# luisdiaz1997/GPzoo

Hardware: AMD Instinct MI355X
Metric: ELBO evals/sec (L=32-latent evaluations, all GPUs) at M=2048 inducing, N=200000, L=32 latents/GPU x 1 GPU(s) (higher is better)
Workload: dtype f32; 1 GPU; BASELINE configs[2]: Slide-seq-shaped synthetic, N=200000 spots, M=2048, L=32 latents/GPU x 1 GPU(s), matern32, f32; latents_total=32, whitened=True, chunk=0, factor_dtype=f64

## Files before the change

gpzoo_amd/csrc/gemmw.hip:

```cpp
#include "gemmw.h"

#include "cov.h"


#include <cmath>
#include <mutex>
#include <type_traits>
#include <utility>

#ifndef GPZ_W_ABL
#define GPZ_W_ABL 0
#endif

namespace gpz {

typedef float f32x4 __attribute__((ext_vector_type(4)));

enum { WB_MEM = 0, WB_GEN = 1 };
enum { WA_DENSE = 0, WA_LOWER = 1, WA_UPPER = 2 };
enum { WE_STORE_STATS = 0,
       WE_STATS = 1,
       WE_STORE = 2,
       WE_STORE_COLSCALE = 3,
       WE_WBAR = 4,
       WE_KBAR = 5,
       WE_ADD_COLSCALE = 6 };

struct WParams {
  const float* A; int64_t lda, sA0;
  const float* B; int64_t ldb, sB0;
  const float* Z; int64_t MD;
  const float* X; int64_t nreal;
  const float* sigma; const float* ell;
  float* C; int64_t ldc, sC0;
  const float* mu; int64_t sMu;
  float* ps_sq; float* ps_mu; int64_t ncols;
  const float* colscale; const float* colvec; int64_t sCs;
  const float* rowvec; int64_t sRv;
  const float* aux;
  int64_t M;
  int L, nblk, mtw, nt, W, strips;
  int pair, colmajor;
  const int32_t* gate;
};

constexpr int W_BK = 16;

template <int TM, int TN, int BSRC, int D>
struct WLds {
  static constexpr int A_ELEMS = TM * W_BK;
  static constexpr int RPP = 256 / TN;
  static constexpr int PITCH = 256 + (RPP == 2 ? 8 : RPP == 1 ? 4 : 16);
  static constexpr int B_ELEMS = (W_BK / RPP) * PITCH;
  static constexpr int STAGE = A_ELEMS + B_ELEMS;
  static constexpr int ZB = 128 * D;
  static constexpr size_t bytes = sizeof(float) * (2 * STAGE + (BSRC == WB_GEN ? 2 * ZB : 0));
};

template <int TM, int TN, int BSRC, int ATRI, int EPI, int KIND, int D>
__global__ __launch_bounds__(64 * (TM / 128) * (TN / 32)) __attribute__((amdgpu_waves_per_eu(4, 4))) void gemmw_kernel(const WParams p) {
  constexpr int BK = W_BK;
  if (p.gate && *p.gate == 0) return;
  constexpr int WMW = TM / 128, WNW = TN / 32;
  constexpr int NW = WMW * WNW;
  static_assert(NW == 8 || NW == 16, "8 or 16 waves of 128 x 32");
  using G = WLds<TM, TN, BSRC, D>;
  constexpr int RPP = G::RPP, PITCH = G::PITCH;
  extern __shared__ __attribute__((aligned(1024))) char smem_raw[];
  float* const smem = reinterpret_cast<float*>(smem_raw);
  auto sA = [&](int buf) -> float* { return smem + buf * G::STAGE; };
  auto sB = [&](int buf) -> float* { return smem + buf * G::STAGE + G::A_ELEMS; };
  float* const sZ = smem + 2 * G::STAGE;
  auto addrB = [](int k, int n) { return (k / RPP) * PITCH + (k % RPP) * TN + n; };

  int tj, b0, leg_ti[2], nlegs = 1;
  {
    const int bid = blockIdx.x;
    const int x = bid & 7, s = bid >> 3;
    if (BSRC == WB_GEN) {
      const int ug = s / p.W, within = s - ug * p.W;
      const int u = ug * 8 + x;
      const int per_level = p.L * p.strips;
      if (u >= p.mtw * per_level) return;
      const int level = u / per_level, rem = u - level * per_level;
      leg_ti[0] = leg_ti[1] = (ATRI == WA_LOWER) ? p.mtw - 1 - level : level;
      b0 = rem / p.strips;
      tj = (rem - b0 * p.strips) * p.W + within;
    } else {
      const int per_unit = (p.pair ? (p.mtw + 1) >> 1 : p.mtw) * p.W;
      const int u = (s / per_unit) * 8 + x, within = s % per_unit;
      if (u >= p.L * p.strips) return;
      b0 = u / p.strips;
      const int nrow = p.pair ? (p.mtw + 1) >> 1 : p.mtw;
      const int pi = p.colmajor ? within % nrow : within / p.W, far = p.pair ? p.mtw - 1 - pi : pi;
      const int strip = u - b0 * p.strips, c0 = strip * p.nt / p.strips, c1 = (strip + 1) * p.nt / p.strips;
      tj = c0 + (p.colmajor ? within / nrow : within % p.W);
      if (tj >= c1) return;
      const bool long_first = ((s >> 5) & 1) == 0;
      leg_ti[0] = ((ATRI == WA_LOWER) == long_first) ? far : pi;
      leg_ti[1] = ((ATRI == WA_LOWER) == long_first) ? pi : far;
      nlegs = far == pi ? 1 : 2;
      if (!p.pair) leg_ti[0] = leg_ti[1] = (ATRI == WA_LOWER) ? p.mtw - 1 - pi : pi;
    }
    if (tj >= p.nt) return;
  }
  const int tid = threadIdx.x, lane = tid & 63;
  const int wave = __builtin_amdgcn_readfirstlane(tid >> 6);
  const int wn = wave % WNW;
  const int r = lane & 15, q = lane >> 4;
  const int Mp = p.nblk * 128;

  typedef __attribute__((address_space(3))) void lds_void;
  constexpr int NPA = TM / (16 * NW);
#if defined(__HIP_DEVICE_COMPILE__)
  const __amdgpu_buffer_rsrc_t a_rsrc = __builtin_amdgcn_make_buffer_rsrc(
      const_cast<float*>(p.A + b0 * p.sA0), 0, (int)(p.lda * Mp * sizeof(float)), 0x00020000);
  const __amdgpu_buffer_rsrc_t b_rsrc = __builtin_amdgcn_make_buffer_rsrc(
      const_cast<float*>(BSRC == WB_MEM ? p.B + b0 * p.sB0 : p.Z), 0,
      (int)((BSRC == WB_MEM ? p.ldb * Mp : p.MD) * sizeof(float)), 0x00020000);
#endif
  auto k_begin_of = [&](int ti) { return (ATRI == WA_UPPER) ? TM * ti : 0; };
  auto k_end_of = [&](int ti) { return (ATRI == WA_LOWER) ? min(TM * (ti + 1), Mp) : Mp; };
  int a_soff[NPA], b_soff = 0;
  auto gperm = [](int w) { const int t = (w >> 2) & 3; return (((t >> 1) ^ t) & 1) << 1 | (t >> 1); };
  const int a_voff = ((lane >> 2) * (int)p.lda + (((lane & 3) ^ gperm(lane >> 2)) * 4)) * (int)sizeof(float);
  const int b_voff = ((lane / (TN / 4)) * (int)p.ldb + (lane % (TN / 4)) * 4) * (int)sizeof(float);
  bool abl_first = true;
  auto stage_load = [&](int buf) __attribute__((always_inline)) {
    if ((GPZ_W_ABL & 2) && !abl_first) return;
    abl_first = false;
#if defined(__HIP_DEVICE_COMPILE__)
#pragma unroll
    for (int h = 0; h < NPA; ++h) {
      __builtin_amdgcn_raw_ptr_buffer_load_lds(a_rsrc, (lds_void*)(sA(buf) + (NPA * wave + h) * 256), 16, a_voff, a_soff[h], 0, 0);
      a_soff[h] += BK * (int)sizeof(float);
    }
    if constexpr (BSRC == WB_MEM) {
      constexpr int NPB = (W_BK / RPP) / NW;
      static_assert(BSRC != WB_MEM || (NPB * NW * RPP == W_BK && NPB >= 1), "whole B pieces per wave");
#pragma unroll
      for (int h = 0; h < NPB; ++h)
        __builtin_amdgcn_raw_ptr_buffer_load_lds(b_rsrc, (lds_void*)(sB(buf) + (wave + NW * h) * PITCH), 16, b_voff,
                                                 b_soff + h * NW * RPP * (int)p.ldb * (int)sizeof(float), 0, 0);
      b_soff += BK * (int)p.ldb * (int)sizeof(float);
    }
#endif
  };
  auto tile_begin = [&](int ti) __attribute__((always_inline)) {
    const int kb = k_begin_of(ti);
#pragma unroll
    for (int h = 0; h < NPA; ++h) {
      int row = ti * TM + (NPA * wave + h) * 16;
      while (row >= Mp) row -= 128;
      a_soff[h] = (row * (int)p.lda + kb) * (int)sizeof(float);
    }
    b_soff = ((kb + RPP * wave) * (int)p.ldb + tj * TN) * (int)sizeof(float);
    stage_load(0);
  };

  constexpr int NXC = TN / 64;
  float xc[NXC][D], ampn[NXC], c0n[NXC], c2n[NXC];
  CovConst cc = {0.f, 0.f, 0.f, 0.f};
  if constexpr (BSRC == WB_GEN) {
    cc = cov_const<KIND>(p.sigma[b0], p.ell[b0]);
#pragma unroll
    for (int h = 0; h < NXC; ++h) {
      const int64_t n = (int64_t)tj * TN + h * 64 + lane;
      const bool real = n < p.nreal;
#pragma unroll
      for (int k = 0; k < D; ++k) xc[h][k] = real ? p.X[n * D + k] : 0.f;
      ampn[h] = real ? cc.amp : 0.f;
      c0n[h] = (KIND != 0 && !real) ? 0.f : cc.c0;
      c2n[h] = real ? cc.c2 : 0.f;
    }
  }
  auto z_load = [&](int blk) __attribute__((always_inline)) {
#if defined(__HIP_DEVICE_COMPILE__)
    if (wave < 2 * D)
      __builtin_amdgcn_raw_ptr_buffer_load_lds(b_rsrc, (lds_void*)(sZ + (blk & 1) * G::ZB + wave * 64), 4, lane * 4,
                                               (blk * G::ZB + wave * 64) * 4, 0, 0);
#endif
  };
  auto b_generate = [&](int buf, int step) __attribute__((always_inline)) {
#pragma unroll
    for (int i = 0; i < BK / NW; ++i) {
      const int kk = wave + NW * i, kg = step * BK + kk;
      const float* zp = sZ + ((kg >> 7) & 1) * G::ZB + (kg & 127) * D;
      float z[D];
#pragma unroll
      for (int k = 0; k < D; ++k) z[k] = zp[k];
#pragma unroll
      for (int h = 0; h < NXC; ++h) {
        const float v = (GPZ_W_ABL & 1) ? z[0] + xc[h][0]
                                        : cov_value<KIND>(cov_radial<KIND>(cov_d2<D>(z, xc[h])), ampn[h], c0n[h], cc.c1, c2n[h]);
        sB(buf)[addrB(kk, h * 64 + lane)] = v;
      }
    }
  };

  f32x4 acc[8][2];

  int wm = 0, nk = 0, db = 0, n_a = 0, fr_a = 0, step0 = 0, t = 0, next_ti = -1;
  bool active = false;
  int fr_b[4];
#pragma unroll
  for (int j = 0; j < 4; ++j) fr_b[j] = addrB(4 * q + j, wn * 32 + r);

  auto mma_step = [&](int buf, auto lo_c, auto hi_c) __attribute__((always_inline)) {
    constexpr int LO = decltype(lo_c)::value, HI = decltype(hi_c)::value;
    float bf[4][2];
#pragma unroll
    for (int j = 0; j < 4; ++j)
#pragma unroll
      for (int ni = 0; ni < 2; ++ni) bf[j][ni] = sB(buf)[fr_b[j] + ni * 16];
#pragma unroll
    for (int half = 0; half < 2; ++half) {
      f32x4 fa[4];
#pragma unroll
      for (int m = 0; m < 4; ++m)
        if (half * 4 + m >= LO && half * 4 + m <= HI)
          fa[m] = *reinterpret_cast<const f32x4*>(sA(buf) + fr_a + (half * 4 + m) * 16 * BK);
#pragma unroll
      for (int j = 0; j < 4; ++j)
#pragma unroll
        for (int m = 0; m < 4; ++m)
#pragma unroll
          for (int ni = 0; ni < 2; ++ni)
            if (half * 4 + m >= LO && half * 4 + m <= HI)
              acc[half * 4 + m][ni] = __builtin_amdgcn_mfma_f32_16x16x4f32(fa[m][j], bf[j][ni], acc[half * 4 + m][ni], 0, 0, 0);
    }
  };

  using std::integral_constant;
  auto step = [&](auto par_c, auto run_c, auto lo_c, auto hi_c) __attribute__((always_inline)) {
    constexpr int P = decltype(par_c)::value;
    if (t + 1 < nk) {
      stage_load(P ^ 1);
      if constexpr (BSRC == WB_GEN) {
        const int st = step0 + t;
        if ((st & 7) == 0 && (st >> 3) + 1 < p.nblk) z_load((st >> 3) + 1);
        b_generate(P ^ 1, st + 1);
      }
    } else if (next_ti >= 0) {
      tile_begin(next_ti);
    }
    if constexpr (decltype(run_c)::value) mma_step(P, lo_c, hi_c);
    if (GPZ_W_ABL & 16) {
      asm volatile("s_waitcnt lgkmcnt(0)" ::: "memory");
      __builtin_amdgcn_s_barrier();
    } else {
      asm volatile("s_waitcnt vmcnt(0)" ::: "memory");
      if (!(GPZ_W_ABL & 8)) __syncthreads();
    }
    ++t;
  };
  using no_run = integral_constant<bool, false>;
  using run = integral_constant<bool, true>;
  using i0 = integral_constant<int, 0>;
  using i1 = integral_constant<int, 1>;
  using i7 = integral_constant<int, 7>;
  auto idle_until = [&](int end) __attribute__((always_inline)) {
    while (t < end) { step(i0{}, no_run{}, i0{}, i7{}); step(i1{}, no_run{}, i0{}, i7{}); }
  };
  auto full_until = [&](int end) __attribute__((always_inline)) {
    while (t < end) { step(i0{}, run{}, i0{}, i7{}); step(i1{}, run{}, i0{}, i7{}); }
  };
  auto diagonal = [&](auto self, auto u_c) __attribute__((always_inline)) -> void {
    constexpr int U = decltype(u_c)::value;
    if constexpr (ATRI == WA_LOWER) step(integral_constant<int, U & 1>{}, run{}, integral_constant<int, U>{}, i7{});
    else step(integral_constant<int, U & 1>{}, run{}, i0{}, integral_constant<int, U>{});
    if constexpr (U + 1 < 8) self(self, integral_constant<int, U + 1>{});
  };

  tile_begin(leg_ti[0]);
#pragma unroll 1
  for (int leg = 0; leg < nlegs; ++leg) {
    const int ti = leg_ti[leg];
    wm = WMW == 1 ? 0 : (wave / WNW) ^ ((ti ^ tj) & 1);
    const int k_begin = k_begin_of(ti);
    nk = (k_end_of(ti) - k_begin) / BK;
    db = WMW * ti + wm;
    active = db < p.nblk && (int64_t)tj * TN + wn * 32 < p.ncols;
    n_a = 8 * (ATRI == WA_LOWER ? db : wm);
    fr_a = (wm * 128 + r) * BK + ((q ^ gperm(r)) * 4);
    step0 = k_begin / BK;
    t = 0;
    next_ti = leg + 1 < nlegs ? leg_ti[leg + 1] : -1;
#pragma unroll
    for (int mi = 0; mi < 8; ++mi)
#pragma unroll
      for (int ni = 0; ni < 2; ++ni) acc[mi][ni] = f32x4{0, 0, 0, 0};
    if constexpr (BSRC == WB_GEN) {
      z_load(step0 >> 3);
      asm volatile("s_waitcnt vmcnt(0)" ::: "memory");
      __syncthreads();
      b_generate(0, step0);
    }
    if (leg == 0) asm volatile("s_waitcnt vmcnt(0)" ::: "memory");
    asm volatile("s_waitcnt lgkmcnt(0)" ::: "memory");
    __builtin_amdgcn_s_barrier();
    if (!active) {
      idle_until(nk);
    } else if constexpr (ATRI == WA_DENSE) {
      full_until(nk);
    } else if constexpr (ATRI == WA_LOWER) {
      full_until(n_a);
      diagonal(diagonal, i0{});
      idle_until(nk);
    } else {
      idle_until(n_a);
      diagonal(diagonal, i0{});
      full_until(nk);
    }

    if (!active) continue;
    if (GPZ_W_ABL & 4) {
      float sum = 0.f;
#pragma unroll
      for (int mi = 0; mi < 8; ++mi)
#pragma unroll
        for (int ni = 0; ni < 2; ++ni)
#pragma unroll
          for (int g = 0; g < 4; ++g) sum += acc[mi][ni][g];
      if (sum == 12345.678f) p.ps_sq[0] = sum;
      continue;
    }
    const int64_t row0 = (int64_t)db * 128;
    const int64_t ccol0 = (int64_t)tj * TN + wn * 32;
    if (BSRC == WB_GEN && row0 + 128 > p.M) {
#pragma unroll
      for (int mi = 0; mi < 8; ++mi)
#pragma unroll
        for (int g = 0; g < 4; ++g)
          if (row0 + mi * 16 + 4 * q + g >= p.M) {
#pragma unroll
            for (int ni = 0; ni < 2; ++ni) acc[mi][ni][g] = 0.f;
          }
    }
    if constexpr (EPI == WE_STORE_STATS || EPI == WE_STATS) {
      float ssq[2] = {0.f, 0.f}, smu[2] = {0.f, 0.f};
#pragma unroll
      for (int mi = 0; mi < 8; ++mi) {
        f32x4 m4 = {0, 0, 0, 0};
        if constexpr (EPI == WE_STORE_STATS) m4 = *reinterpret_cast<const f32x4*>(p.mu + b0 * p.sMu + row0 + 4 * q + mi * 16);
#pragma unroll
        for (int g = 0; g < 4; ++g)
#pragma unroll
          for (int ni = 0; ni < 2; ++ni) {
            const float v = acc[mi][ni][g];
            ssq[ni] = __builtin_fmaf(v, v, ssq[ni]);
            if constexpr (EPI == WE_STORE_STATS) smu[ni] = __builtin_fmaf(m4[g], v, smu[ni]);
          }
      }
#pragma unroll
      for (int ni = 0; ni < 2; ++ni) {
        ssq[ni] += __shfl_xor(ssq[ni], 16); ssq[ni] += __shfl_xor(ssq[ni], 32);
        if constexpr (EPI == WE_STORE_STATS) { smu[ni] += __shfl_xor(smu[ni], 16); smu[ni] += __shfl_xor(smu[ni], 32); }
        if (q == 0) {
          const int64_t o = ((int64_t)b0 * p.nblk + db) * p.ncols + ccol0 + ni * 16 + r;
          p.ps_sq[o] = ssq[ni];
          if constexpr (EPI == WE_STORE_STATS) p.ps_mu[o] = smu[ni];
        }
      }
    }
    if constexpr (EPI != WE_STATS) {
      constexpr int LDE = 36;
      static_assert(NW * 16 * LDE <= G::STAGE, "the epilogue strips fit tile buffer 1");
      float* strip = sA(1) + wave * (16 * LDE);
      float* Cg = p.C + b0 * p.sC0 + row0 * p.ldc + ccol0;
      int srow = lane >> 3;
      asm volatile("" : "+v"(srow));
      const int c4 = (lane & 7) * 4;
      float cs[2] = {1.f, 1.f};
      if constexpr (EPI == WE_STORE_COLSCALE) {
#pragma unroll
        for (int ni = 0; ni < 2; ++ni) cs[ni] = p.colscale[b0 * p.sCs + ccol0 + ni * 16 + r];
      }
      f32x4 sc = {0, 0, 0, 0}, cv = {0, 0, 0, 0};
      if constexpr (EPI == WE_WBAR || EPI == WE_KBAR || EPI == WE_ADD_COLSCALE)
        sc = *reinterpret_cast<const f32x4*>(p.colscale + b0 * p.sCs + ccol0 + c4);
      if constexpr (EPI == WE_WBAR || EPI == WE_KBAR)
        cv = *reinterpret_cast<const f32x4*>(p.colvec + b0 * p.sCs + ccol0 + c4);
#pragma unroll
      for (int mi = 0; mi < 8; ++mi) {
#pragma unroll
        for (int ni = 0; ni < 2; ++ni)
#pragma unroll
          for (int g = 0; g < 4; ++g) strip[(4 * q + g) * LDE + ni * 16 + r] = cs[ni] * acc[mi][ni][g];
        __builtin_amdgcn_wave_barrier();
        f32x4 w[2];
        float rv[2];
        if constexpr (EPI == WE_WBAR || EPI == WE_KBAR || EPI == WE_ADD_COLSCALE) {
#pragma unroll
          for (int it = 0; it < 2; ++it) {
            const int64_t row = mi * 16 + it * 8 + srow;
            if constexpr (EPI == WE_WBAR) w[it] = *reinterpret_cast<const f32x4*>(p.aux + b0 * p.sC0 + (row0 + row) * p.ldc + ccol0 + c4);
            if constexpr (EPI == WE_ADD_COLSCALE) w[it] = *reinterpret_cast<const f32x4*>(Cg + (int64_t)row * p.ldc + c4);
            if constexpr (EPI != WE_ADD_COLSCALE) rv[it] = p.rowvec[b0 * p.sRv + row0 + row];
          }
        }
#pragma unroll
        for (int it = 0; it < 2; ++it) {
          const int row = it * 8 + srow;
          f32x4 v = *reinterpret_cast<const f32x4*>(strip + row * LDE + c4);
          if constexpr (EPI == WE_WBAR) {
#pragma unroll
            for (int e = 0; e < 4; ++e) v[e] = v[e] + rv[it] * cv[e] - w[it][e] * sc[e];
          }
          if constexpr (EPI == WE_KBAR) {
#pragma unroll
            for (int e = 0; e < 4; ++e) v[e] = v[e] * sc[e] + rv[it] * cv[e];
          }
          if constexpr (EPI == WE_ADD_COLSCALE) {
#pragma unroll
            for (int e = 0; e < 4; ++e) v[e] = w[it][e] + v[e] * sc[e];
          }
          *reinterpret_cast<f32x4*>(Cg + (int64_t)(mi * 16 + row) * p.ldc + c4) = v;
        }
        __builtin_amdgcn_wave_barrier();
      }
    }
  }
}

struct NTParams {
  const float* A; const float* B; float* C;
  int64_t ld, sAB, ldc, sC;
  int K, nblk, mt, L, T;
  int S, Ks;
  float* part; int64_t sPart;
  const float* w; int64_t sW;
  const int32_t* gate;
  const float* gm; float* vpart;
};

template <int TM, bool WTS>
__global__ __launch_bounds__(TM * 2) __attribute__((amdgpu_waves_per_eu(4, 4))) void gemmw_nt_kernel(const NTParams p) {
  constexpr int BK = W_BK, TN = 128;
  if (p.gate && *p.gate == 0) return;
  constexpr int NW = TM / 32;
  constexpr int A_ELEMS = TM * BK, B_ELEMS = TN * BK, STAGE = A_ELEMS + B_ELEMS;
  extern __shared__ __attribute__((aligned(1024))) char smem_raw[];
  float* const smem = reinterpret_cast<float*>(smem_raw);
  auto sA = [&](int buf) -> float* { return smem + buf * STAGE; };
  auto sB = [&](int buf) -> float* { return smem + buf * STAGE + A_ELEMS; };
  int b0, ti, tj, piece;
  {
    const int nb = (int)gridDim.x, qn = nb >> 3, rem = nb & 7, x = blockIdx.x & 7;
    const int lid0 = x * qn + min(x, rem) + (int)(blockIdx.x >> 3);
    const int grp = lid0 / p.T;
    const int t = lid0 - grp * p.T;
    b0 = grp / p.S;
    piece = grp - b0 * p.S;
    if constexpr (TM == 256) {
      int i = (int)((sqrtf(4.0f * (float)t + 1.0f) - 1.0f) * 0.5f);
      while ((i + 1) * (i + 2) <= t) ++i;
      while (i * (i + 1) > t) --i;
      ti = i; tj = t - i * (i + 1);
    } else {
      int i = (int)((sqrtf(8.0f * (float)t + 1.0f) - 1.0f) * 0.5f);
      while ((i + 1) * (i + 2) / 2 <= t) ++i;
      while (i * (i + 1) / 2 > t) --i;
      ti = i; tj = t - i * (i + 1) / 2;
    }
  }
  const int tid = threadIdx.x, lane = tid & 63;
  const int wave = __builtin_amdgcn_readfirstlane(tid >> 6);
  const int wm = wave >> 2, wn = wave & 3;
  const int r = lane & 15, q = lane >> 4;
  const int Mp = p.nblk * 128;
  const int db = (TM / 128) * ti + wm;
  const bool active = db < p.nblk && tj <= db;
  const bool same = TM == 128 && p.A == p.B && tj == ti;
  typedef __attribute__((address_space(3))) void lds_void;
#if defined(__HIP_DEVICE_COMPILE__)
  const __amdgpu_buffer_rsrc_t a_rsrc = __builtin_amdgcn_make_buffer_rsrc(
      const_cast<float*>(p.A + b0 * p.sAB), 0, (int)(p.ld * Mp * sizeof(float)), 0x00020000);
  const __amdgpu_buffer_rsrc_t b_rsrc = __builtin_amdgcn_make_buffer_rsrc(
      const_cast<float*>(p.B + b0 * p.sAB), 0, (int)(p.ld * Mp * sizeof(float)), 0x00020000);
#endif
  auto gperm = [](int w) { const int t = (w >> 2) & 3; return (((t >> 1) ^ t) & 1) << 1 | (t >> 1); };
  const int voff = ((lane >> 2) * (int)p.ld + (((lane & 3) ^ gperm(lane >> 2)) * 4)) * (int)sizeof(float);
  int a_soff[2], b_soff;
#pragma unroll
  for (int h = 0; h < 2; ++h) {
    int row = ti * TM + (2 * wave + h) * 16;
    while (row >= Mp) row -= 128;
    a_soff[h] = (row * (int)p.ld + piece * p.Ks) * (int)sizeof(float);
  }
  constexpr int NPB = 8 / NW;
  b_soff = ((tj * TN + wave * NPB * 16) * (int)p.ld + piece * p.Ks) * (int)sizeof(float);
  auto stage_load = [&](int buf) __attribute__((always_inline)) {
#if defined(__HIP_DEVICE_COMPILE__)
#pragma unroll
    for (int h = 0; h < 2; ++h) {
      __builtin_amdgcn_raw_ptr_buffer_load_lds(a_rsrc, (lds_void*)(sA(buf) + (2 * wave + h) * 256), 16, voff, a_soff[h], 0, 0);
      a_soff[h] += BK * (int)sizeof(float);
    }
    if (!same) {
#pragma unroll
      for (int h = 0; h < NPB; ++h)
        __builtin_amdgcn_raw_ptr_buffer_load_lds(b_rsrc, (lds_void*)(sB(buf) + (wave * NPB + h) * 256), 16, voff,
                                                 b_soff + h * 16 * (int)p.ld * (int)sizeof(float), 0, 0);
      b_soff += BK * (int)sizeof(float);
    }
#endif
  };
  const float* wk = WTS ? p.w + b0 * p.sW + (int64_t)piece * p.Ks + 4 * (lane >> 4) : nullptr;
  f32x4 wv;
  auto w_load = [&]() __attribute__((always_inline)) {
    if constexpr (WTS) { wv = *reinterpret_cast<const f32x4*>(wk); wk += BK; }
  };
  const int fr_a = (wm * 128 + r) * BK + ((q ^ gperm(r)) * 4);
  const int nk = (min(p.K, (piece + 1) * p.Ks) - piece * p.Ks) / BK;
  const bool split = p.S > 1;
  const bool diag = WTS && p.A == p.B && db == tj && db < p.nblk;
  if (diag) {
    auto diag_path = [&](auto wn_c) __attribute__((always_inline)) {
      constexpr int C0 = decltype(wn_c)::value, C1 = 7 - C0, N0 = 8 - C0, N1 = 8 - C1;
      const bool rd = p.gm != nullptr;
      const float* gk = rd ? p.gm + b0 * p.sW + (int64_t)piece * p.Ks + 4 * (lane >> 4) : nullptr;
      f32x4 gv = f32x4{0, 0, 0, 0};
      float pv0 = 0.f, pv1 = 0.f;
      f32x4 a0[N0], a1[N1];
#pragma unroll
      for (int i = 0; i < N0; ++i) a0[i] = f32x4{0, 0, 0, 0};
#pragma unroll
      for (int i = 0; i < N1; ++i) a1[i] = f32x4{0, 0, 0, 0};
      const int fb_off = r * BK + ((q ^ gperm(r)) * 4) + (same ? -A_ELEMS : 0);
      auto step = [&](int buf, bool more) __attribute__((always_inline)) {
        f32x4 f0 = *reinterpret_cast<const f32x4*>(sB(buf) + fb_off + C0 * 16 * BK);
        f32x4 f1 = *reinterpret_cast<const f32x4*>(sB(buf) + fb_off + C1 * 16 * BK);
        f0 *= wv; f1 *= wv;
        if (more) w_load();
#pragma unroll
        for (int mi = C0; mi < 8; ++mi) {
          const f32x4 fa = *reinterpret_cast<const f32x4*>(sA(buf) + fr_a + mi * 16 * BK);
#pragma unroll
          for (int j = 0; j < 4; ++j) {
            a0[mi - C0] = __builtin_amdgcn_mfma_f32_16x16x4f32(fa[j], f0[j], a0[mi - C0], 0, 0, 0);
            if (mi >= C1) a1[mi >= C1 ? mi - C1 : 0] = __builtin_amdgcn_mfma_f32_16x16x4f32(fa[j], f1[j], a1[mi >= C1 ? mi - C1 : 0], 0, 0, 0);
          }
          if (mi == 2 * C0 || mi == 2 * C0 + 1) {
            if (rd) {
              const f32x4 t = fa * gv;
              if (mi == 2 * C0) pv0 += (t[0] + t[1]) + (t[2] + t[3]); else pv1 += (t[0] + t[1]) + (t[2] + t[3]);
            }
          }
        }
        if (more && rd) { gv = *reinterpret_cast<const f32x4*>(gk); gk += BK; }
      };
      if (rd) { gv = *reinterpret_cast<const f32x4*>(gk); gk += BK; }
      stage_load(0);
      w_load();
      asm volatile("s_waitcnt vmcnt(0)" ::: "memory");
      __syncthreads();
      for (int t = 0; t < nk; t += 2) {
        if (t + 1 < nk) stage_load(1);
        step(0, t + 1 < nk);
        asm volatile("s_waitcnt vmcnt(0)" ::: "memory");
        __syncthreads();
        if (t + 2 < nk) stage_load(0);
        step(1, t + 2 < nk);
        asm volatile("s_waitcnt vmcnt(0)" ::: "memory");
        __syncthreads();
      }
      if (rd) {
        float* vp = p.vpart + ((int64_t)piece * p.L + b0) * Mp + db * 128;
        pv0 += __shfl_xor(pv0, 16); pv0 += __shfl_xor(pv0, 32);
        pv1 += __shfl_xor(pv1, 16); pv1 += __shfl_xor(pv1, 32);
        if (q == 0) { vp[(2 * C0) * 16 + r] = pv0; vp[(2 * C0 + 1) * 16 + r] = pv1; }
      }
      float* Cg = (split ? p.part + piece * p.sPart : p.C) + b0 * p.sC + (int64_t)db * 128 * p.ldc + (int64_t)tj * TN;
      auto put = [&](const f32x4& a, int mi, int c) __attribute__((always_inline)) {
        float* o = Cg + (int64_t)(mi * 16 + 4 * q) * p.ldc + c * 16 + r;
#pragma unroll
        for (int g = 0; g < 4; ++g) o[g * p.ldc] = split ? a[g] : o[g * p.ldc] + a[g];
      };
#pragma unroll
      for (int mi = C0; mi < 8; ++mi) put(a0[mi - C0], mi, C0);
#pragma unroll
      for (int mi = C1; mi < 8; ++mi) put(a1[mi - C1], mi, C1);
    };
    switch (wn) {
      case 0: diag_path(std::integral_constant<int, 0>{}); break;
      case 1: diag_path(std::integral_constant<int, 1>{}); break;
      case 2: diag_path(std::integral_constant<int, 2>{}); break;
      default: diag_path(std::integral_constant<int, 3>{}); break;
    }
    return;
  }
  f32x4 acc[8][2];
#pragma unroll
  for (int mi = 0; mi < 8; ++mi)
#pragma unroll
    for (int ni = 0; ni < 2; ++ni) acc[mi][ni] = f32x4{0, 0, 0, 0};
  const int fr_b = (wn * 32 + r) * BK + ((q ^ gperm(r)) * 4) + (same ? -A_ELEMS : 0);
  auto mma_step = [&](int buf, bool more) __attribute__((always_inline)) {
    f32x4 fb[2];
#pragma unroll
    for (int ni = 0; ni < 2; ++ni) {
      fb[ni] = *reinterpret_cast<const f32x4*>(sB(buf) + fr_b + ni * 16 * BK);
      if constexpr (WTS) fb[ni] *= wv;
    }
    if (more) w_load();
#pragma unroll
    for (int half = 0; half < 2; ++half) {
      f32x4 fa[4];
#pragma unroll
      for (int m = 0; m < 4; ++m) fa[m] = *reinterpret_cast<const f32x4*>(sA(buf) + fr_a + (half * 4 + m) * 16 * BK);
#pragma unroll
      for (int j = 0; j < 4; ++j)
#pragma unroll
        for (int m = 0; m < 4; ++m)
#pragma unroll
          for (int ni = 0; ni < 2; ++ni)
            acc[half * 4 + m][ni] = __builtin_amdgcn_mfma_f32_16x16x4f32(fa[m][j], fb[ni][j], acc[half * 4 + m][ni], 0, 0, 0);
    }
  };
  stage_load(0);
  w_load();
  asm volatile("s_waitcnt vmcnt(0)" ::: "memory");
  __syncthreads();
  if (active) {
    for (int t = 0; t < nk; t += 2) {
      if (t + 1 < nk) stage_load(1);
      mma_step(0, t + 1 < nk);
      asm volatile("s_waitcnt vmcnt(0)" ::: "memory");
      __syncthreads();
      if (t + 2 < nk) stage_load(0);
      mma_step(1, t + 2 < nk);
      asm volatile("s_waitcnt vmcnt(0)" ::: "memory");
      __syncthreads();
    }
  } else {
    for (int t = 0; t < nk; t += 2) {
      if (t + 1 < nk) stage_load(1);
      asm volatile("s_waitcnt vmcnt(0)" ::: "memory");
      __syncthreads();
      if (t + 2 < nk) stage_load(0);
      asm volatile("s_waitcnt vmcnt(0)" ::: "memory");
      __syncthreads();
    }
    return;
  }
  constexpr int LDE = 36;
  float* strip = smem + wave * (32 * LDE);
  float* Cg = (split ? p.part + piece * p.sPart : p.C) + b0 * p.sC + (int64_t)db * 128 * p.ldc + (int64_t)tj * TN + wn * 32;
  const int srow = lane >> 3, c4 = (lane & 7) * 4;
#pragma unroll
  for (int pass = 0; pass < 4; ++pass) {
#pragma unroll
    for (int mm = 0; mm < 2; ++mm)
#pragma unroll
      for (int ni = 0; ni < 2; ++ni)
#pragma unroll
        for (int g = 0; g < 4; ++g) strip[(mm * 16 + 4 * q + g) * LDE + ni * 16 + r] = acc[pass * 2 + mm][ni][g];
    __builtin_amdgcn_wave_barrier();
    f32x4 cin[4];
#pragma unroll
    for (int it = 0; it < 4; ++it)
      cin[it] = split ? f32x4{0, 0, 0, 0} : *reinterpret_cast<const f32x4*>(Cg + (int64_t)(pass * 32 + it * 8 + srow) * p.ldc + c4);
#pragma unroll
    for (int it = 0; it < 4; ++it) {
      const int row = it * 8 + srow;
      const f32x4 v = *reinterpret_cast<const f32x4*>(strip + row * LDE + c4);
      *reinterpret_cast<f32x4*>(Cg + (int64_t)(pass * 32 + row) * p.ldc + c4) = cin[it] + v;
    }
    __builtin_amdgcn_wave_barrier();
  }
}

__global__ __launch_bounds__(256) void nt_reduce_kernel(float* __restrict__ C, const float* __restrict__ part, int S, int64_t sPart,
                                                        int Mp, int64_t total4, const int32_t* __restrict__ gate, int sym) {
  const int64_t i4 = (int64_t)blockIdx.x * 256 + threadIdx.x;
  if (i4 >= total4 || (gate && *gate == 0)) return;
  const int64_t e = i4 * 4;
  const int col = (int)(e % Mp), row = (int)((e / Mp) % Mp);
  if ((col >> 7) > (row >> 7) || (sym && (col >> 4) > (row >> 4))) return;
  f32x4 v = *reinterpret_cast<const f32x4*>(C + e);
  for (int s = 0; s < S; ++s) v += *reinterpret_cast<const f32x4*>(part + s * sPart + e);
  *reinterpret_cast<f32x4*>(C + e) = v;
}

__global__ __launch_bounds__(256) void nt_vsum_kernel(const float* __restrict__ vpart, int S, int64_t LM, double* __restrict__ v,
                                                      int64_t Mp, int64_t v_stride) {
  const int64_t i = (int64_t)blockIdx.x * 256 + threadIdx.x;
  if (i >= LM) return;
  double t = 0.0;
  for (int s = 0; s < S; ++s) t += (double)vpart[s * LM + i];
  v[(i / Mp) * v_stride + i % Mp] = t;
}

template <typename K>
static int launch_wide(K kernel, size_t lds, const WParams& p, int64_t nblocks, hipStream_t s, int threads = 512) {
  struct Seen { const void* fn; int dev; };
  static Seen seen[64];
  static int n_seen = 0;
  static std::mutex mu;
  int dev = 0;
  GPZ_HIP_OK(hipGetDevice(&dev));
  if (lds > 64 * 1024) {
    const void* fn = reinterpret_cast<const void*>(kernel);
    std::lock_guard<std::mutex> lock(mu);
    bool have = false;
    for (int i = 0; i < n_seen; ++i) have = have || (seen[i].fn == fn && seen[i].dev == dev);
    if (!have) {
      GPZ_HIP_OK(hipFuncSetAttribute(fn, hipFuncAttributeMaxDynamicSharedMemorySize, (int)lds));
      if (n_seen < 64) seen[n_seen++] = Seen{fn, dev};
    }
  }
  GPZ_REQUIRE(nblocks > 0 && nblocks < (1ll << 31), "wide product: bad grid");
  hipLaunchKernelGGL(kernel, dim3((unsigned)nblocks), dim3((unsigned)threads), lds, s, p);
  GPZ_LAUNCH_OK();
  return 0;
}

bool fused1_supported(int dtype, int kind, int d) {
  return dtype == GPZ_F32 && (d == 1 || d == 2) &&
         (kind == GPZ_KERNEL_RBF || kind == GPZ_KERNEL_MATERN32 || kind == GPZ_KERNEL_MATERN12 || kind == GPZ_KERNEL_MATERN52);
}

int fused1_launch(const Fused1Args& a, hipStream_t s) {
  GPZ_REQUIRE(fused1_supported(GPZ_F32, a.kind, a.d), "fused stage 1: kind=%d d=%d unsupported", a.kind, a.d);
  GPZ_REQUIRE(a.Mp % 128 == 0 && a.ncp % 128 == 0 && a.Mp > 0 && a.ncp > 0 && a.L > 0, "fused stage 1: bad extents");
  GPZ_REQUIRE(a.Mp * a.Mp * 4 < (1ll << 31) && a.M * a.d * 4 < (1ll << 31), "fused stage 1: M too large");
  constexpr int TM = 512, TN = 128;
  WParams p = {};
  p.A = a.Linv; p.lda = a.Mp; p.sA0 = a.Mp * a.Mp;
  p.Z = a.Z; p.MD = a.M * a.d; p.M = a.M;
  p.X = a.X; p.nreal = a.nreal;
  p.sigma = a.sigma; p.ell = a.ell;
  p.C = a.Wt; p.ldc = a.ncp; p.sC0 = a.Mp * a.ncp;
  p.mu = a.muE; p.sMu = a.Mp;
  p.ps_sq = a.ps_sq; p.ps_mu = a.ps_mu; p.ncols = a.ncp;
  p.L = a.L; p.nblk = (int)(a.Mp / 128); p.mtw = (int)((a.Mp + TM - 1) / TM); p.nt = (int)(a.ncp / TN);
  int strips = (p.nt + 31) / 32;
  const int want = (32 + p.mtw * p.L - 1) / (p.mtw * p.L);
  if (strips < want) strips = want < p.nt ? want : p.nt;
  p.W = (p.nt + strips - 1) / strips;
  p.strips = (p.nt + p.W - 1) / p.W;
  const int64_t units = (int64_t)p.mtw * p.L * p.strips;
  const int64_t nblocks = (units + 7) / 8 * 8 * p.W;
#define GPZ_W1(KIND, D) return launch_wide(gemmw_kernel<TM, TN, WB_GEN, WA_LOWER, WE_STORE_STATS, KIND, D>, \
                                           WLds<TM, TN, WB_GEN, D>::bytes, p, nblocks, s, 1024)
  if (a.kind == GPZ_KERNEL_MATERN32) { if (a.d == 2) GPZ_W1(1, 2); GPZ_W1(1, 1); }
  if (a.kind == GPZ_KERNEL_MATERN12) { if (a.d == 2) GPZ_W1(4, 2); GPZ_W1(4, 1); }
  if (a.kind == GPZ_KERNEL_MATERN52) { if (a.d == 2) GPZ_W1(5, 2); GPZ_W1(5, 1); }
  if (a.d == 2) GPZ_W1(0, 2);
  GPZ_W1(0, 1);
#undef GPZ_W1
}

bool wide_product_supported(int64_t Mp, int64_t ncp) {
  return Mp % 128 == 0 && ncp % 128 == 0 && Mp * Mp * 4 < (1ll << 31) && Mp * ncp * 4 < (1ll << 31);
}

template <int TM, int TN>
static int wide_product_launch_t(const WideArgs& a, hipStream_t s) {
  WParams p = {};
  p.A = a.A; p.lda = a.Mp; p.sA0 = a.Mp * a.Mp;
  p.B = a.B; p.ldb = a.ncp; p.sB0 = a.Mp * a.ncp;
  p.C = a.C; p.ldc = a.ncp; p.sC0 = a.Mp * a.ncp;
  p.mu = a.mu; p.sMu = a.Mp;
  p.ps_sq = a.ps_sq; p.ps_mu = a.ps_mu; p.ncols = a.ncp; p.M = a.Mp;
  p.colscale = a.colscale; p.colvec = a.colvec; p.sCs = a.ncp; p.rowvec = a.rowvec; p.sRv = a.Mp; p.aux = a.aux;
  p.gate = a.gate;
  p.L = a.L; p.nblk = (int)(a.Mp / 128); p.mtw = (int)((a.Mp + TM - 1) / TM); p.nt = (int)((a.ncp + TN - 1) / TN);
  constexpr int WMAX = 4096 / TN;
  int strips = (p.nt + WMAX - 1) / WMAX;
  const int want = (8 + p.L - 1) / p.L;
  if (strips < want) strips = want < p.nt ? want : p.nt;
  p.strips = strips;
  p.W = (p.nt + strips - 1) / strips;
  const int64_t units = (int64_t)p.L * p.strips;
  const int64_t paired = (units + 7) / 8 * 8 * ((p.mtw + 1) / 2) * p.W;
  p.pair = p.colmajor = paired >= 4 * 512;
  const int64_t nblocks = p.pair ? paired : (units + 7) / 8 * 8 * p.mtw * p.W;
  constexpr size_t lds = WLds<TM, TN, WB_MEM, 1>::bytes;
#define GPZ_WM(ATRI, EPI) return launch_wide(gemmw_kernel<TM, TN, WB_MEM, ATRI, EPI, 0, 1>, lds, p, nblocks, s)
  switch (a.epilogue) {
    case WIDE_STORE_STATS:
      GPZ_REQUIRE(!a.upper && a.C && a.mu && a.ps_sq && a.ps_mu, "wide product: store + statistics is the lower-triangular product and needs C, mu and both slabs");
      GPZ_WM(WA_LOWER, WE_STORE_STATS);
    case WIDE_STATS:
      GPZ_REQUIRE(a.upper && a.ps_sq, "wide product: statistics only is the upper-triangular product");
      GPZ_WM(WA_UPPER, WE_STATS);
    case WIDE_STORE:
      GPZ_REQUIRE(a.upper && a.C, "wide product: the plain store is built for the upper-triangular product");
      GPZ_WM(WA_UPPER, WE_STORE);
    case WIDE_STORE_COLSCALE:
      GPZ_REQUIRE(a.upper && a.C && a.colscale, "wide product: the column-scaled store is the upper-triangular product and needs the factors");
      GPZ_WM(WA_UPPER, WE_STORE_COLSCALE);
    case WIDE_WBAR:
      GPZ_REQUIRE(!a.upper && a.C && a.colscale && a.colvec && a.rowvec && a.aux, "wide product: the W-bar epilogue needs its operands");
      GPZ_WM(WA_LOWER, WE_WBAR);
    case WIDE_KBAR:
      GPZ_REQUIRE(a.upper == 2 && a.C && a.colscale && a.colvec && a.rowvec, "wide product: the K-bar epilogue is the dense product and needs its vectors");
      GPZ_WM(WA_DENSE, WE_KBAR);
    case WIDE_ADD_COLSCALE:
      GPZ_REQUIRE(a.upper == 1 && a.C && a.colscale, "wide product: the accumulating column-scaled store is the upper-triangular product");
      GPZ_WM(WA_UPPER, WE_ADD_COLSCALE);
    default: break;
  }
#undef GPZ_WM
  GPZ_REQUIRE(false, "wide product: unknown epilogue %d", a.epilogue);
}

int wide_product_launch(const WideArgs& a, hipStream_t s) {
  GPZ_REQUIRE(wide_product_supported(a.Mp, a.ncp) && a.L > 0, "wide product: bad extents");
  return wide_product_launch_t<128, 256>(a, s);
}

bool wide_nt_supported(int64_t Mp, int64_t K) {
  return Mp % 128 == 0 && K % 128 == 0 && K > 0 && Mp * K * 4 < (1ll << 31);
}

static bool nt_small_tiles(int64_t nblk) { return nblk <= 4; }
static int64_t nt_tiles(int64_t nblk) {
  if (nt_small_tiles(nblk)) return nblk * (nblk + 1) / 2;
  const int64_t mt = (nblk + 1) / 2;
  return mt * (mt + 1) - (nblk & 1);
}

int wide_nt_pieces(int64_t Mp, int64_t K, int L) {
  const int64_t tiles = nt_tiles(Mp / 128) * L;
  if (tiles >= 384) {
    const double r = (double)tiles / 512.0;
    int best = 1;
    double best_cost = 1e30;
    for (int S = 1; S <= 4; ++S) {
      if (S > 1 && K / S < 2048) break;
      const double rounds = r * S, cost = std::ceil(rounds - 1e-9) / rounds * (1.0 + 0.015 * (S - 1));
      if (cost < best_cost - 1e-9) { best_cost = cost; best = S; }
    }
    return best;
  }
  int64_t S = (nt_small_tiles(Mp / 128) ? 1024 : 512) / tiles;
  S = std::min<int64_t>(S, K / 1024);
  S = std::min<int64_t>(S, 16);
  return (int)std::max<int64_t>(S, 1);
}

size_t wide_nt_vpart_floats(int64_t Mp, int64_t K, int L) { return (size_t)wide_nt_pieces(Mp, K, L) * L * Mp; }

size_t wide_nt_scratch_floats(int64_t Mp, int64_t K, int L) {
  const int S = wide_nt_pieces(Mp, K, L);
  return S > 1 ? (size_t)S * L * Mp * Mp : 0;
}

int wide_nt_launch(const float* A, const float* B, float* C, int64_t Mp, int64_t K, int L, hipStream_t s, float* scratch,
                   const float* w, const int32_t* gate, const float* gm, float* vpart, double* v, int64_t v_stride) {
  GPZ_REQUIRE(A && B && C && wide_nt_supported(Mp, K) && L > 0, "wide A B^T: bad arguments");
  GPZ_REQUIRE(!gm || (w && vpart && v && A == B), "wide A B^T: the row products A gm need weights, A == B and their buffers");
  NTParams p;
  p.w = w; p.sW = K; p.gate = gate; p.gm = gm; p.vpart = vpart;
  p.A = A; p.B = B; p.C = C; p.ld = K; p.sAB = Mp * K; p.ldc = Mp; p.sC = Mp * Mp;
  p.K = (int)K; p.nblk = (int)(Mp / 128); p.mt = (p.nblk + 1) / 2; p.L = L;
  const bool small = nt_small_tiles(p.nblk);
  p.T = (int)nt_tiles(p.nblk);
  int S = scratch ? wide_nt_pieces(Mp, K, L) : 1;
  p.Ks = (int)(((K + S - 1) / S + 31) / 32 * 32);
  S = (int)((K + p.Ks - 1) / p.Ks);
  p.S = S; p.part = scratch; p.sPart = (int64_t)L * Mp * Mp;
  const int64_t nblocks = (int64_t)p.T * L * S;
  GPZ_REQUIRE(nblocks > 0 && nblocks < (1ll << 31), "wide A B^T: bad grid");
  if (small) {
    constexpr size_t lds = sizeof(float) * 2 * (128 + 128) * W_BK;
    if (w) hipLaunchKernelGGL((gemmw_nt_kernel<128, true>), dim3((unsigned)nblocks), dim3(256), lds, s, p);
    else hipLaunchKernelGGL((gemmw_nt_kernel<128, false>), dim3((unsigned)nblocks), dim3(256), lds, s, p);
  } else {
    constexpr size_t lds = sizeof(float) * 2 * (256 + 128) * W_BK;
    if (w) hipLaunchKernelGGL((gemmw_nt_kernel<256, true>), dim3((unsigned)nblocks), dim3(512), lds, s, p);
    else hipLaunchKernelGGL((gemmw_nt_kernel<256, false>), dim3((unsigned)nblocks), dim3(512), lds, s, p);
  }
  GPZ_LAUNCH_OK();
  if (S > 1) {
    const int64_t total4 = (int64_t)L * Mp * Mp / 4;
    hipLaunchKernelGGL(nt_reduce_kernel, dim3((unsigned)((total4 + 255) / 256)), dim3(256), 0, s, C, scratch, S, p.sPart, (int)Mp, total4, gate, (int)(w != nullptr && A == B));
    GPZ_LAUNCH_OK();
  }
  if (gm) {
    const int64_t LM = (int64_t)L * Mp;
    hipLaunchKernelGGL(nt_vsum_kernel, dim3((unsigned)((LM + 255) / 256)), dim3(256), 0, s, vpart, S, LM, v, Mp, v_stride);
    GPZ_LAUNCH_OK();
  }
  return 0;
}

}
```

Baseline: 2.647 ELBO evals/s.

## Schedule symmetric weighted NT GEMM as banded full tiles plus paired 128-wide halves

```diff
diff --git a/gpzoo_amd/csrc/gemmw.hip b/gpzoo_amd/csrc/gemmw.hip
--- a/gpzoo_amd/csrc/gemmw.hip
+++ b/gpzoo_amd/csrc/gemmw.hip
@@ -4,6 +4,8 @@
 
 
 #include <cmath>
+#include <cstdlib>
+#include <cstring>
 #include <mutex>
 #include <type_traits>
 #include <utility>
@@ -432,40 +434,26 @@
   const float* w; int64_t sW;
   const int32_t* gate;
   const float* gm; float* vpart;
+  int band;
 };
 
+constexpr int NT_HALF_FLOATS = 2 * (128 + 128) * W_BK;
+
 template <int TM, bool WTS>
-__global__ __launch_bounds__(TM * 2) __attribute__((amdgpu_waves_per_eu(4, 4))) void gemmw_nt_kernel(const NTParams p) {
+__device__ __attribute__((always_inline)) void nt_tile(const NTParams& p, float* const smem, const int wave, const int b0,
+                                                        const int piece, const int ti, const int tj, const bool idle) {
   constexpr int BK = W_BK, TN = 128;
-  if (p.gate && *p.gate == 0) return;
   constexpr int NW = TM / 32;
   constexpr int A_ELEMS = TM * BK, B_ELEMS = TN * BK, STAGE = A_ELEMS + B_ELEMS;
-  extern __shared__ __attribute__((aligned(1024))) char smem_raw[];
-  float* const smem = reinterpret_cast<float*>(smem_raw);
+  const int nk = (min(p.K, (piece + 1) * p.Ks) - piece * p.Ks) / BK;
+  if (idle) {
+    __syncthreads();
+    for (int t = 0; t < nk; t += 2) { __syncthreads(); __syncthreads(); }
+    return;
+  }
   auto sA = [&](int buf) -> float* { return smem + buf * STAGE; };
   auto sB = [&](int buf) -> float* { return smem + buf * STAGE + A_ELEMS; };
-  int b0, ti, tj, piece;
-  {
-    const int nb = (int)gridDim.x, qn = nb >> 3, rem = nb & 7, x = blockIdx.x & 7;
-    const int lid0 = x * qn + min(x, rem) + (int)(blockIdx.x >> 3);
-    const int grp = lid0 / p.T;
-    const int t = lid0 - grp * p.T;
-    b0 = grp / p.S;
-    piece = grp - b0 * p.S;
-    if constexpr (TM == 256) {
-      int i = (int)((sqrtf(4.0f * (float)t + 1.0f) - 1.0f) * 0.5f);
-      while ((i + 1) * (i + 2) <= t) ++i;
-      while (i * (i + 1) > t) --i;
-      ti = i; tj = t - i * (i + 1);
-    } else {
-      int i = (int)((sqrtf(8.0f * (float)t + 1.0f) - 1.0f) * 0.5f);
-      while ((i + 1) * (i + 2) / 2 <= t) ++i;
-      while (i * (i + 1) / 2 > t) --i;
-      ti = i; tj = t - i * (i + 1) / 2;
-    }
-  }
-  const int tid = threadIdx.x, lane = tid & 63;
-  const int wave = __builtin_amdgcn_readfirstlane(tid >> 6);
+  const int lane = threadIdx.x & 63;
   const int wm = wave >> 2, wn = wave & 3;
   const int r = lane & 15, q = lane >> 4;
   const int Mp = p.nblk * 128;
@@ -512,7 +500,6 @@
     if constexpr (WTS) { wv = *reinterpret_cast<const f32x4*>(wk); wk += BK; }
   };
   const int fr_a = (wm * 128 + r) * BK + ((q ^ gperm(r)) * 4);
-  const int nk = (min(p.K, (piece + 1) * p.Ks) - piece * p.Ks) / BK;
   const bool split = p.S > 1;
   const bool diag = WTS && p.A == p.B && db == tj && db < p.nblk;
   if (diag) {
@@ -669,6 +656,65 @@
     }
     __builtin_amdgcn_wave_barrier();
   }
+}
+
+template <int TM, bool WTS>
+__global__ __launch_bounds__(TM * 2) __attribute__((amdgpu_waves_per_eu(4, 4))) void gemmw_nt_kernel(const NTParams p) {
+  if (p.gate && *p.gate == 0) return;
+  extern __shared__ __attribute__((aligned(1024))) char smem_raw[];
+  float* const smem = reinterpret_cast<float*>(smem_raw);
+  const int wave = __builtin_amdgcn_readfirstlane((int)threadIdx.x >> 6);
+  int b0, ti, tj, piece;
+  bool halves = false, idle = false;
+  {
+    const int nb = (int)gridDim.x, qn = nb >> 3, rem = nb & 7, x = blockIdx.x & 7;
+    const int lid0 = x * qn + min(x, rem) + (int)(blockIdx.x >> 3);
+    const int grp = lid0 / p.T;
+    const int t = lid0 - grp * p.T;
+    b0 = grp / p.S;
+    piece = grp - b0 * p.S;
+    if (TM == 256 && WTS && p.band) {
+      const int mtf = p.nblk >> 1, nf = mtf * (mtf - 1);
+      if (t < nf) {
+        int i = (int)((sqrtf(4.0f * (float)t + 1.0f) + 1.0f) * 0.5f);
+        while ((i + 1) * i <= t) ++i;
+        while (i * (i - 1) > t) --i;
+        ti = i; tj = t - i * (i - 1);
+      } else {
+        halves = true;
+        const int nfull = mtf + ((p.nblk & 1) ? p.nblk - 1 : 0), nfp = (nfull + 1) >> 1;
+        const int u = t - nf, h = wave >> 2;
+        if (u < nfp) {
+          const int f = 2 * u + h;
+          idle = f >= nfull;
+          ti = f < mtf ? 2 * f + 1 : p.nblk - 1;
+          tj = f < mtf ? 2 * f : f - mtf;
+        } else {
+          const int d = 2 * (u - nfp) + h;
+          idle = d >= p.nblk;
+          ti = tj = d;
+        }
+        if (idle) ti = tj = 0;
+      }
+    } else if constexpr (TM == 256) {
+      int i = (int)((sqrtf(4.0f * (float)t + 1.0f) - 1.0f) * 0.5f);
+      while ((i + 1) * (i + 2) <= t) ++i;
+      while (i * (i + 1) > t) --i;
+      ti = i; tj = t - i * (i + 1);
+    } else {
+      int i = (int)((sqrtf(8.0f * (float)t + 1.0f) - 1.0f) * 0.5f);
+      while ((i + 1) * (i + 2) / 2 <= t) ++i;
+      while (i * (i + 1) / 2 > t) --i;
+      ti = i; tj = t - i * (i + 1) / 2;
+    }
+  }
+  if constexpr (TM == 256 && WTS) {
+    if (halves) {
+      nt_tile<128, WTS>(p, smem + (wave >> 2) * NT_HALF_FLOATS, wave & 3, b0, piece, ti, tj, idle);
+      return;
+    }
+  }
+  nt_tile<TM, WTS>(p, smem, wave, b0, piece, ti, tj, false);
 }
 
 __global__ __launch_bounds__(256) void nt_reduce_kernel(float* __restrict__ C, const float* __restrict__ part, int S, int64_t sPart,
@@ -823,6 +869,16 @@
   return mt * (mt + 1) - (nblk & 1);
 }
 
+static int64_t nt_band_units(int64_t nblk) {
+  const int64_t mtf = nblk / 2, nfull = mtf + ((nblk & 1) ? nblk - 1 : 0);
+  return mtf * (mtf - 1) + (nfull + 1) / 2 + (nblk + 1) / 2;
+}
+
+static bool nt_band_enabled() {
+  static const bool on = [] { const char* e = std::getenv("GPZ_NT_BAND"); return !(e && !std::strcmp(e, "0")); }();
+  return on;
+}
+
 int wide_nt_pieces(int64_t Mp, int64_t K, int L) {
   const int64_t tiles = nt_tiles(Mp / 128) * L;
   if (tiles >= 384) {
@@ -858,7 +914,8 @@
   p.A = A; p.B = B; p.C = C; p.ld = K; p.sAB = Mp * K; p.ldc = Mp; p.sC = Mp * Mp;
   p.K = (int)K; p.nblk = (int)(Mp / 128); p.mt = (p.nblk + 1) / 2; p.L = L;
   const bool small = nt_small_tiles(p.nblk);
-  p.T = (int)nt_tiles(p.nblk);
+  p.band = !small && w && A == B && nt_band_enabled();
+  p.T = (int)(p.band ? nt_band_units(p.nblk) : nt_tiles(p.nblk));
   int S = scratch ? wide_nt_pieces(Mp, K, L) : 1;
   p.Ks = (int)(((K + S - 1) / S + 31) / 32 * 32);
   S = (int)((K + p.Ks - 1) / p.Ks);
@@ -870,7 +927,7 @@
     if (w) hipLaunchKernelGGL((gemmw_nt_kernel<128, true>), dim3((unsigned)nblocks), dim3(256), lds, s, p);
     else hipLaunchKernelGGL((gemmw_nt_kernel<128, false>), dim3((unsigned)nblocks), dim3(256), lds, s, p);
   } else {
-    constexpr size_t lds = sizeof(float) * 2 * (256 + 128) * W_BK;
+    const size_t lds = sizeof(float) * (p.band ? 2 * NT_HALF_FLOATS : 2 * (256 + 128) * W_BK);
     if (w) hipLaunchKernelGGL((gemmw_nt_kernel<256, true>), dim3((unsigned)nblocks), dim3(512), lds, s, p);
     else hipLaunchKernelGGL((gemmw_nt_kernel<256, false>), dim3((unsigned)nblocks), dim3(512), lds, s, p);
   }
```

After: 2.646 ELBO evals/s. About the same (-0.0%).

## Split wide symmetric A B^T into off-diagonal 256-row and diagonal-band 128-row launches

Applied to the files above, without the earlier changes.

```diff
diff --git a/gpzoo_amd/csrc/gemmw.hip b/gpzoo_amd/csrc/gemmw.hip
--- a/gpzoo_amd/csrc/gemmw.hip
+++ b/gpzoo_amd/csrc/gemmw.hip
@@ -423,10 +423,12 @@
   }
 }
 
+enum { NT_MAP_ALL = 0, NT_MAP_FULL = 1, NT_MAP_BAND = 2 };
 struct NTParams {
   const float* A; const float* B; float* C;
   int64_t ld, sAB, ldc, sC;
   int K, nblk, mt, L, T;
+  int map;
   int S, Ks;
   float* part; int64_t sPart;
   const float* w; int64_t sW;
@@ -453,10 +455,20 @@
     b0 = grp / p.S;
     piece = grp - b0 * p.S;
     if constexpr (TM == 256) {
-      int i = (int)((sqrtf(4.0f * (float)t + 1.0f) - 1.0f) * 0.5f);
-      while ((i + 1) * (i + 2) <= t) ++i;
-      while (i * (i + 1) > t) --i;
-      ti = i; tj = t - i * (i + 1);
+      if (p.map == NT_MAP_FULL) {
+        int i = (int)((sqrtf(4.0f * (float)t + 1.0f) + 1.0f) * 0.5f);
+        while (i * (i + 1) <= t) ++i;
+        while (i * (i - 1) > t) --i;
+        ti = i; tj = t - i * (i - 1);
+      } else {
+        int i = (int)((sqrtf(4.0f * (float)t + 1.0f) - 1.0f) * 0.5f);
+        while ((i + 1) * (i + 2) <= t) ++i;
+        while (i * (i + 1) > t) --i;
+        ti = i; tj = t - i * (i + 1);
+      }
+    } else if (p.map == NT_MAP_BAND) {
+      const int i = t / 3, m = t - 3 * i;
+      ti = 2 * i + (m > 0); tj = 2 * i + (m > 1);
     } else {
       int i = (int)((sqrtf(8.0f * (float)t + 1.0f) - 1.0f) * 0.5f);
       while ((i + 1) * (i + 2) / 2 <= t) ++i;
@@ -671,13 +683,16 @@
   }
 }
 
-__global__ __launch_bounds__(256) void nt_reduce_kernel(float* __restrict__ C, const float* __restrict__ part, int S, int64_t sPart,
-                                                        int Mp, int64_t total4, const int32_t* __restrict__ gate, int sym) {
+__global__ __launch_bounds__(256) void nt_reduce_kernel(float* __restrict__ C, const float* __restrict__ part, int S, int Sfull,
+                                                        int64_t sPart, int Mp, int64_t total4, const int32_t* __restrict__ gate,
+                                                        int sym) {
   const int64_t i4 = (int64_t)blockIdx.x * 256 + threadIdx.x;
   if (i4 >= total4 || (gate && *gate == 0)) return;
   const int64_t e = i4 * 4;
   const int col = (int)(e % Mp), row = (int)((e / Mp) % Mp);
   if ((col >> 7) > (row >> 7) || (sym && (col >> 4) > (row >> 4))) return;
+  if ((col >> 8) < (row >> 8)) S = Sfull;
+  if (S <= 1) return;
   f32x4 v = *reinterpret_cast<const f32x4*>(C + e);
   for (int s = 0; s < S; ++s) v += *reinterpret_cast<const f32x4*>(part + s * sPart + e);
   *reinterpret_cast<f32x4*>(C + e) = v;
@@ -823,10 +838,9 @@
   return mt * (mt + 1) - (nblk & 1);
 }
 
-int wide_nt_pieces(int64_t Mp, int64_t K, int L) {
-  const int64_t tiles = nt_tiles(Mp / 128) * L;
-  if (tiles >= 384) {
-    const double r = (double)tiles / 512.0;
+static int nt_pieces_rule(int64_t tiles, int64_t K, int64_t resident, int64_t once) {
+  if (tiles >= resident * 3 / 4) {
+    const double r = (double)tiles / (double)resident;
     int best = 1;
     double best_cost = 1e30;
     for (int S = 1; S <= 4; ++S) {
@@ -836,16 +850,41 @@
     }
     return best;
   }
-  int64_t S = (nt_small_tiles(Mp / 128) ? 1024 : 512) / tiles;
+  int64_t S = once / tiles;
   S = std::min<int64_t>(S, K / 1024);
   S = std::min<int64_t>(S, 16);
   return (int)std::max<int64_t>(S, 1);
 }
 
-size_t wide_nt_vpart_floats(int64_t Mp, int64_t K, int L) { return (size_t)wide_nt_pieces(Mp, K, L) * L * Mp; }
+int wide_nt_pieces(int64_t Mp, int64_t K, int L) {
+  return nt_pieces_rule(nt_tiles(Mp / 128) * L, K, 512, nt_small_tiles(Mp / 128) ? 1024 : 512);
+}
+
+static int64_t nt_full_tiles(int64_t nblk) { const int64_t mt = (nblk + 1) / 2; return mt * (mt - 1); }
+static int64_t nt_band_tiles(int64_t nblk) { return 3 * (nblk / 2) + (nblk & 1); }
+static int nt_full_pieces(int64_t Mp, int64_t K, int L) { return nt_pieces_rule(nt_full_tiles(Mp / 128) * L, K, 512, 512); }
+static int nt_band_pieces(int64_t Mp, int64_t K, int L) { return nt_pieces_rule(nt_band_tiles(Mp / 128) * L, K, 1024, 1024); }
+
+static int g_nt_split_mode = 0;
+static bool nt_split(int64_t Mp, int64_t K, int L) {
+  if (nt_small_tiles(Mp / 128) || g_nt_split_mode == 1) return false;
+  if (g_nt_split_mode == 2) return true;
+  return nt_band_tiles(Mp / 128) * L >= 768;
+}
+
+static int nt_most_pieces(int64_t Mp, int64_t K, int L, bool with_full) {
+  int S = wide_nt_pieces(Mp, K, L);
+  if (!nt_small_tiles(Mp / 128)) {
+    S = std::max(S, nt_band_pieces(Mp, K, L));
+    if (with_full) S = std::max(S, nt_full_pieces(Mp, K, L));
+  }
+  return S;
+}
+
+size_t wide_nt_vpart_floats(int64_t Mp, int64_t K, int L) { return (size_t)nt_most_pieces(Mp, K, L, false) * L * Mp; }
 
 size_t wide_nt_scratch_floats(int64_t Mp, int64_t K, int L) {
-  const int S = wide_nt_pieces(Mp, K, L);
+  const int S = nt_most_pieces(Mp, K, L, true);
   return S > 1 ? (size_t)S * L * Mp * Mp : 0;
 }
 
@@ -857,27 +896,41 @@
   p.w = w; p.sW = K; p.gate = gate; p.gm = gm; p.vpart = vpart;
   p.A = A; p.B = B; p.C = C; p.ld = K; p.sAB = Mp * K; p.ldc = Mp; p.sC = Mp * Mp;
   p.K = (int)K; p.nblk = (int)(Mp / 128); p.mt = (p.nblk + 1) / 2; p.L = L;
-  const bool small = nt_small_tiles(p.nblk);
-  p.T = (int)nt_tiles(p.nblk);
-  int S = scratch ? wide_nt_pieces(Mp, K, L) : 1;
-  p.Ks = (int)(((K + S - 1) / S + 31) / 32 * 32);
-  S = (int)((K + p.Ks - 1) / p.Ks);
-  p.S = S; p.part = scratch; p.sPart = (int64_t)L * Mp * Mp;
-  const int64_t nblocks = (int64_t)p.T * L * S;
-  GPZ_REQUIRE(nblocks > 0 && nblocks < (1ll << 31), "wide A B^T: bad grid");
-  if (small) {
-    constexpr size_t lds = sizeof(float) * 2 * (128 + 128) * W_BK;
-    if (w) hipLaunchKernelGGL((gemmw_nt_kernel<128, true>), dim3((unsigned)nblocks), dim3(256), lds, s, p);
-    else hipLaunchKernelGGL((gemmw_nt_kernel<128, false>), dim3((unsigned)nblocks), dim3(256), lds, s, p);
+  p.part = scratch; p.sPart = (int64_t)L * Mp * Mp;
+  const bool small = nt_small_tiles(p.nblk), two = nt_split(Mp, K, L);
+  auto launch = [&](int map, int64_t tiles, int pieces, bool wave4, int* S_out) -> int {
+    p.map = map; p.T = (int)tiles;
+    int S = scratch ? pieces : 1;
+    p.Ks = (int)(((K + S - 1) / S + 31) / 32 * 32);
+    S = (int)((K + p.Ks - 1) / p.Ks);
+    p.S = S;
+    const int64_t nblocks = (int64_t)p.T * L * S;
+    GPZ_REQUIRE(nblocks > 0 && nblocks < (1ll << 31), "wide A B^T: bad grid");
+    if (wave4) {
+      constexpr size_t lds = sizeof(float) * 2 * (128 + 128) * W_BK;
+      if (w) hipLaunchKernelGGL((gemmw_nt_kernel<128, true>), dim3((unsigned)nblocks), dim3(256), lds, s, p);
+      else hipLaunchKernelGGL((gemmw_nt_kernel<128, false>), dim3((unsigned)nblocks), dim3(256), lds, s, p);
+    } else {
+      constexpr size_t lds = sizeof(float) * 2 * (256 + 128) * W_BK;
+      if (w) hipLaunchKernelGGL((gemmw_nt_kernel<256, true>), dim3((unsigned)nblocks), dim3(512), lds, s, p);
+      else hipLaunchKernelGGL((gemmw_nt_kernel<256, false>), dim3((unsigned)nblocks), dim3(512), lds, s, p);
+    }
+    GPZ_LAUNCH_OK();
+    *S_out = S;
+    return 0;
+  };
+  int S = 1, Sfull = 1;
+  if (two) {
+    if (int rc = launch(NT_MAP_FULL, nt_full_tiles(p.nblk), nt_full_pieces(Mp, K, L), false, &Sfull)) return rc;
+    if (int rc = launch(NT_MAP_BAND, nt_band_tiles(p.nblk), nt_band_pieces(Mp, K, L), true, &S)) return rc;
   } else {
-    constexpr size_t lds = sizeof(float) * 2 * (256 + 128) * W_BK;
-    if (w) hipLaunchKernelGGL((gemmw_nt_kernel<256, true>), dim3((unsigned)nblocks), dim3(512), lds, s, p);
-    else hipLaunchKernelGGL((gemmw_nt_kernel<256, false>), dim3((unsigned)nblocks), dim3(512), lds, s, p);
-  }
-  GPZ_LAUNCH_OK();
-  if (S > 1) {
+    if (int rc = launch(NT_MAP_ALL, nt_tiles(p.nblk), wide_nt_pieces(Mp, K, L), small, &S)) return rc;
+    Sfull = S;
+  }
+  if (S > 1 || Sfull > 1) {
     const int64_t total4 = (int64_t)L * Mp * Mp / 4;
-    hipLaunchKernelGGL(nt_reduce_kernel, dim3((unsigned)((total4 + 255) / 256)), dim3(256), 0, s, C, scratch, S, p.sPart, (int)Mp, total4, gate, (int)(w != nullptr && A == B));
+    hipLaunchKernelGGL(nt_reduce_kernel, dim3((unsigned)((total4 + 255) / 256)), dim3(256), 0, s, C, scratch, S, Sfull, p.sPart,
+                       (int)Mp, total4, gate, (int)(w != nullptr && A == B));
     GPZ_LAUNCH_OK();
   }
   if (gm) {
@@ -889,3 +942,9 @@
 }
 
 }
+
+extern "C" int gpz_debug_nt_split(int mode) {
+  const int prev = gpz::g_nt_split_mode;
+  if (mode >= 0 && mode <= 2) gpz::g_nt_split_mode = mode;
+  return prev;
+}
```

Result: no change. 2.661 ELBO evals/s before, 2.659 ELBO evals/s after (-0.1%).
